# lfilipozzi/PathPlanning

Measured on AMD Instinct MI355X. Metric: hybrid_astar_plans_per_sec_1024x1024, higher is better.
Workload: dtype f64

## Files before the change

### pathplanning_amd/csrc/pp_internal.hpp

```cpp
#pragma once

#include <hip/hip_runtime.h>
#include <stdint.h>
#include <string>
#include <vector>

#include "../../include/pp_hip.h"
#include "pp_device.hpp"

namespace pph {

void set_error(const std::string& msg);
int hip_fail(hipError_t e, const char* what);

#define PP_HIP_TRY(expr)                       \
	do {                                       \
		hipError_t _e = (expr);                \
		if (_e != hipSuccess)                  \
			return pph::hip_fail(_e, #expr);   \
	} while (0)

constexpr int kMaxPrimitives = 128;
struct PrimTable {
	int n;
	double kappa[kMaxPrimitives];
	double invKappa[kMaxPrimitives];
	int8_t backward[kMaxPrimitives];
};

struct RolloutParams {
	double arcLength;
	double spatialRes, angularRes;
	ppd::Resolutions lat;
	double forwardMult, reverseMult, voronoiMult;
	float voroDiagRes;
	int headingAlias;
};

struct NonHoloDesc {
	int nx, ny, na;
	double spatialRes, angularRes, offX, offY;
	double rmin;
	float reverseCost, forwardCost, switchCost;
	double minMult;
	int negativeKRead;
};

hipError_t launch_d2_to_distance(hipStream_t s, const int32_t* d2, float* dist, int64_t n, float res);
hipError_t launch_occ_to_u8(hipStream_t s, const int32_t* occ, uint8_t* occ8, int64_t n);
hipError_t launch_check_states(hipStream_t s, const ppd::MapView& m, int64_t n, const double* poses, uint8_t* valid);
hipError_t launch_check_states_fused(hipStream_t s, const ppd::MapView& m, int64_t n, uint64_t seed, uint64_t* count);
hipError_t launch_check_arcs(hipStream_t s, const ppd::MapView& m, int64_t n, const double* from, const double* kappa, const double* length, const int32_t* dir,
	uint8_t* valid, float* last);
hipError_t launch_check_segments(hipStream_t s, const ppd::MapView& m, int64_t n, const double* from, const double* to, uint8_t* valid);
hipError_t launch_rollout(hipStream_t s, const ppd::MapView& m, const RolloutParams& rp, const PrimTable& prims, int64_t nParents, const double* parents,
	uint8_t* valid, double* pose, int32_t* key, double* cost, double* length);
hipError_t launch_rs_solve(hipStream_t s, int64_t n, const double* from, const double* to, double rmin, float rev, float fwd, float sw, int32_t* word,
	double* tuv, float* cost, double* segLength);
hipError_t launch_valid_bits(hipStream_t s, const float* dist, int64_t cells, float minSafeRadius, uint32_t* bits);
hipError_t launch_nonholo_build(hipStream_t s, const NonHoloDesc& d, double* table);
hipError_t launch_knn(hipStream_t s, int64_t nPoints, const double* pts, int64_t nQueries, const double* q, int k, int32_t* idx, double* d2);

struct WavefrontWorkspace;
int64_t wavefront_workspace_bytes(int rows, int cols);
int wavefront_resident_blocks();
hipError_t warm_up_wavefront(hipStream_t s, const ppd::MapView& m, int32_t* ctlDev);
constexpr int kSlotBits = 20;
constexpr uint32_t kSlotMask = (1u << kSlotBits) - 1u;
constexpr uint32_t kGenMask = (1u << (31 - kSlotBits)) - 1u;
struct WavefrontPublish {
	const int32_t* slotList = nullptr;
	unsigned long long* readyTail = nullptr;
	unsigned long long* ready = nullptr;
	unsigned long long readyMask = 0;
	int* goalCounter = nullptr;
	int* exitCounter = nullptr;
	unsigned long long* urgent = nullptr;
	unsigned long long* urgentHead = nullptr;
	unsigned long long urgentMask = 0;
	int* claimed = nullptr;
	const uint64_t* occBits = nullptr;
	uint32_t* tilesQueue = nullptr;
	int tilesQueueWaves = 0;
	int* tilesCtl = nullptr;
	int32_t* tilesFallback = nullptr;
	unsigned long long* tilesStats = nullptr;
	hipStream_t fallbackStream = nullptr;
	hipEvent_t fallbackEvent = nullptr;
	const int* nGoalsDev = nullptr;
	int* resetOnExit = nullptr;
	bool agentPoseLoads = false;
};
void occ_bits_dims(int rows, int cols, int& wpr, int& nWordRows);
hipError_t launch_occ_bits(hipStream_t s, const uint8_t* occ8, int rows, int cols, uint64_t* bits);
bool wavefront_tiles_supported(int rows, int cols);
int wavefront_tiles_resident_blocks(int rows, int cols);
size_t wavefront_tiles_queue_words(int rows, int cols);
hipError_t warm_up_wavefront_tiles(hipStream_t s, const ppd::MapView& m, int* ctlDev);
hipError_t launch_wavefront_tiles(hipStream_t s, const ppd::MapView& m, int nGoals, const int32_t* goalCellsDev, float* costDev, bool tiledOut, const double* goalPosesDev,
	const double* orderStartsDev, float* orderKeysDev, const WavefrontPublish& pub);
hipError_t launch_order_by_key(hipStream_t s, int n, const float* keysDev, int32_t* orderOutDev);
bool wavefront_tiles_enabled();
hipError_t launch_wavefront(hipStream_t s, const ppd::MapView& m, int nGoals, const int32_t* goalCellsDev, float* costDev, void* workspaceDev,
	int64_t workspaceBytesPerSlot, int nSlots, int32_t* errorFlagDev, unsigned long long* profDev = nullptr, bool tiledOut = false,
	const double* goalPosesDev = nullptr, bool countersZeroed = false, const double* orderStartsDev = nullptr, int32_t* orderOutDev = nullptr,
	int* doneCounterDev = nullptr, float* orderKeysDev = nullptr, const WavefrontPublish& pub = WavefrontPublish());

}

struct pp_ctx;
struct pp_map;
namespace pph {
struct GvdReference;
void gvd_reference_free(pp_map* map);
int refresh_occupancy_views(pp_map* map, hipStream_t s);
void ctx_release(pp_ctx* ctx);
void map_release(pp_map* map);
}

struct pp_ctx {
	int refs = 1;
	int device = 0;
	hipStream_t stream = nullptr;
	bool ownsStream = false;
	hipEvent_t ev0 = nullptr, ev1 = nullptr;
// ... 27 lines not shown
```

### pathplanning_amd/csrc/pp_pipeline.hpp

```cpp
#pragma once

#include <chrono>
#include <cstring>
#include <deque>
#include <unordered_map>

namespace {

__global__ void __launch_bounds__(256) k_pipe_scatter(int n, const int32_t* __restrict__ slotList, const double* __restrict__ startsIn, const double* __restrict__ goalsIn,
	const uint64_t* __restrict__ seedsIn, double* __restrict__ starts, double* __restrict__ goals, uint64_t* __restrict__ seeds, MapView m, float urgentClearance, PipeCtl* ctl,
	unsigned long long* __restrict__ urgent, unsigned long long urgentMask, int* __restrict__ claimed)
{
	const int i = (int)(blockIdx.x * blockDim.x + threadIdx.x);
	bool isUrgent = false;
	uint32_t entry = 0;
	if (i < n) {
		entry = (uint32_t)slotList[i];
		const size_t s = (size_t)(entry & pph::kSlotMask);
		for (int k = 0; k < 3; k++) {
			starts[3 * s + k] = startsIn[3 * (size_t)i + k];
			goals[3 * s + k] = goalsIn[3 * (size_t)i + k];
		}
		seeds[s] = seedsIn[i];
		if (claimed) {
// ... 574 lines not shown
		P->segmentEvents.pop_back();
	} else {
		PP_HIP_TRY(hipEventCreateWithFlags(&seg.done, hipEventDisableTiming));
	}
	struct DeadGuard {
		pp_pipeline* P;
		bool armed = true;
		~DeadGuard()
		{
			if (armed)
				P->dead = true;
		}
	} guard { P };
	P->segmentEvents.push_back(seg.done);
	int32_t* const stage = P->slotStage + P->slotListPos;
	int32_t* const listDev = P->slotLists + P->slotListPos;
	P->slotListPos += (size_t)k;
	for (int i = 0; i < k; i++) {
		const int32_t s = P->freeSlots.back();
		P->freeSlots.pop_back();
		uint32_t& gen = P->slotGen[(size_t)s];
		gen = gen >= pph::kGenMask ? 1u : gen + 1u;
		stage[i] = (int32_t)((uint32_t)s | (gen << pph::kSlotBits));
		P->slotState[(size_t)s] = 1;
		const uint64_t ticket = P->nTickets++;
		P->ticketOfSlot[(size_t)s] = ticket;
		P->slotOfTicket[ticket] = s;
		if (tickets_out)
			tickets_out[i] = ticket;
	}
	hipStream_t const w = P->wfStream[P->nextWf];
	const int wfIdx = P->nextWf;
	int32_t* const wctl = P->wfCtl[P->nextWf];
	const int fbSet = P->nextFbSet;
	P->nextFbSet = (P->nextFbSet + 1) % pp_pipeline::kFbSets;
	if (P->fbUsed[fbSet])
		PP_HIP_TRY(hipEventSynchronize(P->fbDone[fbSet]));
	int32_t* const werr = P->errFlags + P->nextWf;
	const bool tilesOn = pl->map->occBits && pph::wavefront_tiles_enabled() && pph::wavefront_tiles_supported(pl->map->desc.rows, pl->map->desc.cols);
	void* const wws = P->wfWorkspace[tilesOn ? 0 : P->nextWf];
	P->nextWf = (P->nextWf + 1) % P->nWf;
	PP_HIP_TRY(hipMemcpyAsync(listDev, stage, (size_t)k * 4, hipMemcpyHostToDevice, P->ctlStream));
	pl->args.m = pl->map->view();
	hipLaunchKernelGGL(k_pipe_scatter, dim3((k + 255) / 256), dim3(256), 0, P->ctlStream, k, listDev, starts_dev, goals_dev, seeds_dev, pl->dStarts, pl->dGoals, pl->dSeeds, pl->args.m,
		P->urgentClearance < 0.0f ? 2.0f * pl->args.m.minSafeRadius : P->urgentClearance, P->ctl, P->urgent, P->readyMask, P->claimed);
	PP_HIP_TRY(hipGetLastError());
	PP_HIP_TRY(hipEventRecord(P->evIngest, P->ctlStream));
	PP_HIP_TRY(hipStreamSynchronize(P->ctlStream));
	PP_HIP_TRY(hipStreamWaitEvent(w, P->evIngest, 0));
	pl->args.m = pl->map->view();
	pph::WavefrontPublish pub;
	pub.slotList = listDev;
	pub.readyTail = &P->ctl->readyTail;
	pub.ready = P->ready;
	pub.readyMask = P->readyMask;
	pub.goalCounter = wctl + 1;
	pub.exitCounter = wctl + 2;
	pub.claimed = P->claimed;
	pub.occBits = pl->map->occBits;
	pub.tilesCtl = P->fbCtl[fbSet];
	pub.tilesFallback = P->fbList[fbSet];
	pub.tilesQueue = P->tilesQueue[wfIdx];
	pub.tilesQueueWaves = P->tilesQueue[wfIdx] ? P->tilesQueueWaves : 0;
	pub.fallbackStream = P->fbStream;
	pub.fallbackEvent = P->fbAfterTiles[fbSet];
	if (P->urgentClearance != 0.0f) {
		pub.urgent = P->urgent;
		pub.urgentHead = &P->ctl->urgentHead;
		pub.urgentMask = P->readyMask;
	}
	const pp_pipeline::Timed tm = timed_take(P, w, 0, k);
	PP_HIP_TRY(pph::launch_wavefront(w, pl->args.m, k, nullptr, pl->costFields, wws, pl->wfBytesPerSlot, P->wfBlocks, werr, nullptr, true, pl->dGoals,
		true, nullptr, nullptr, nullptr, nullptr, pub));
	timed_done(P, w, tm);
	PP_HIP_TRY(hipEventRecord(P->fbDone[fbSet], P->fbStream));
	P->fbUsed[fbSet] = true;
	PP_HIP_TRY(hipEventRecord(seg.done, w));
	P->segmentEvents.pop_back();
	P->segments.push_back(seg);
	P->nSubmitted += (unsigned long long)k;
	*n_accepted = k;
	const int rc = pipe_launch_search(P);
	guard.armed = rc != PP_OK;
	return rc;
}

int pp_pipeline_submit(pp_pipeline* P, int32_t n_queries, const double* starts_host, const double* goals_host, const uint64_t* seeds_host, uint64_t* tickets_out, int32_t* n_accepted)
{
	if (!P || n_queries < 0 || !n_accepted || (n_queries > 0 && (!starts_host || !goals_host || !seeds_host))) {
		set_error("invalid arguments");
		return PP_ERR_INVALID;
	}
	*n_accepted = 0;
	int k = n_queries < (int)P->freeSlots.size() ? n_queries : (int)P->freeSlots.size();
	if (k == 0)
		return PP_OK;
	PP_HIP_TRY(hipSetDevice(P->pl->map->ctx->device));
	double *ds = nullptr, *dg = nullptr;
	uint64_t* dz = nullptr;
	hipError_t e = hipMalloc((void**)&ds, (size_t)k * 24);
	if (e == hipSuccess)
		e = hipMalloc((void**)&dg, (size_t)k * 24);
	if (e == hipSuccess)
		e = hipMalloc((void**)&dz, (size_t)k * 8);
	if (e == hipSuccess)
		e = hipMemcpy(ds, starts_host, (size_t)k * 24, hipMemcpyHostToDevice);
// ... 216 lines not shown
```

### pathplanning_amd/csrc/pp_wavefront_tiles.hip

```cpp
#include <cstdio>
#include "pp_internal.hpp"

#include <cstdlib>
#include <type_traits>

using namespace ppd;

namespace {

constexpr int TT = 64;
template <int TW>
struct TileShape {
	static constexpr int LS = TW + 2;
	static constexpr int LN = (TT + 2) * LS;
	static constexpr int LNP = (LN + 3) & ~3;
	typedef typename std::conditional<TW == 64, uint64_t, uint32_t>::type Mask;
};
constexpr uint32_t kInfBits = 0x7F800000u;
#ifndef PP_WF_TILES_PRIO_DEFAULT
#define PP_WF_TILES_PRIO_DEFAULT 1
#endif
#ifndef PP_WF_TILE_WIDTH_DEFAULT
#define PP_WF_TILE_WIDTH_DEFAULT 32
#endif

__device__ __forceinline__ void wave_sync()
{
	__builtin_amdgcn_fence(__ATOMIC_ACQ_REL, "wavefront");
	__builtin_amdgcn_wave_barrier();
}
__device__ __forceinline__ uint32_t from_prev_lane(uint32_t v, uint32_t first) { return (uint32_t)__builtin_amdgcn_update_dpp((int)first, (int)v, 0x138, 0xF, 0xF, false); }
__device__ __forceinline__ uint32_t from_next_lane(uint32_t v, uint32_t last) { return (uint32_t)__builtin_amdgcn_update_dpp((int)last, (int)v, 0x130, 0xF, 0xF, false); }
__device__ __forceinline__ uint64_t from_prev_lane64(uint64_t v, uint64_t first)
{
	return (uint64_t)from_prev_lane((uint32_t)v, (uint32_t)first) | ((uint64_t)from_prev_lane((uint32_t)(v >> 32), (uint32_t)(first >> 32)) << 32);
}
__device__ __forceinline__ uint64_t from_next_lane64(uint64_t v, uint64_t last)
{
	return (uint64_t)from_next_lane((uint32_t)v, (uint32_t)last) | ((uint64_t)from_next_lane((uint32_t)(v >> 32), (uint32_t)(last >> 32)) << 32);
}
__device__ __forceinline__ uint32_t mask_from_prev(uint32_t v, uint32_t first) { return from_prev_lane(v, first); }
__device__ __forceinline__ uint32_t mask_from_next(uint32_t v, uint32_t last) { return from_next_lane(v, last); }
__device__ __forceinline__ uint64_t mask_from_prev(uint64_t v, uint64_t first) { return from_prev_lane64(v, first); }
__device__ __forceinline__ uint64_t mask_from_next(uint64_t v, uint64_t last) { return from_next_lane64(v, last); }
__device__ __forceinline__ uint32_t wave_min_u32(uint32_t v)
{
	const int id = (int)0xFFFFFFFF;
	uint32_t x = v;
	x = min(x, (uint32_t)__builtin_amdgcn_update_dpp(id, (int)x, 0x111, 0xF, 0xF, false));
	x = min(x, (uint32_t)__builtin_amdgcn_update_dpp(id, (int)x, 0x112, 0xF, 0xF, false));
	x = min(x, (uint32_t)__builtin_amdgcn_update_dpp(id, (int)x, 0x114, 0xF, 0xF, false));
	x = min(x, (uint32_t)__builtin_amdgcn_update_dpp(id, (int)x, 0x118, 0xF, 0xF, false));
	x = min(x, (uint32_t)__builtin_amdgcn_update_dpp(id, (int)x, 0x142, 0xA, 0xF, false));
	x = min(x, (uint32_t)__builtin_amdgcn_update_dpp(id, (int)x, 0x143, 0xC, 0xF, false));
	return (uint32_t)__builtin_amdgcn_readlane((int)x, 63);
}
__device__ __forceinline__ float wave_min_nonneg(float v) { return __uint_as_float(wave_min_u32(__float_as_uint(v))); }

template <int TW>
__device__ __forceinline__ void tile_cell(int tiledOut, int e, int& i, int& j)
{
	if (tiledOut) {
		const int ft = e >> (2 * kFieldTileLog2), within = e & ((1 << (2 * kFieldTileLog2)) - 1);
		constexpr int perRow = TW >> kFieldTileLog2;
		i = ((ft / perRow) << kFieldTileLog2) + (within >> kFieldTileLog2);
		j = ((ft % perRow) << kFieldTileLog2) + (within & kFieldTileMask);
	} else {
		i = e / TW;
		j = e % TW;
	}
}

__global__ void __launch_bounds__(256) k_occ_bits(const uint8_t* __restrict__ occ8, int rows, int cols, int wpr, int nWordRows, uint64_t* __restrict__ bits)
{
	const int64_t w = (int64_t)blockIdx.x * 4 + (threadIdx.x >> 6);
	const int lane = threadIdx.x & 63;
	if (w >= (int64_t)nWordRows * wpr)
		return;
	const int pr = (int)(w / wpr), pw = (int)(w - (int64_t)pr * wpr);
	const int r = pr - 1, c = (pw - 1) * 64 + lane;
	bool o = true;
	if (r >= 0 && r < rows && pw >= 1 && c < cols)
		o = occ8[(int64_t)r * cols + c] != 0;
	const uint64_t b = __ballot(o);
	if (lane == 0)
		bits[w] = b;
}

struct TilesArgs {
	MapView m;
	int nGoals;
	const int32_t* goalCells;
	const double* goalPoses;
	float* costOut;
	int tiledOut;
	int* ctl;
	int32_t* fbList;
	const double* orderStarts;
	float* orderKeys;
	unsigned long long* stats;
	int forceFallbackEvery;
	int ldsPerWave;
	int prio;
	pph::WavefrontPublish pub;
};

template <int TW, bool kProf, bool kGQ>
__global__ void __launch_bounds__(512) k_wavefront_tiles(TilesArgs A)
{
	unsigned long long ph[5] = { 0, 0, 0, 0, 0 }, tl = 0;
#define TILE_STAMP(i)                                        \
	if (kProf) {                                             \
		const unsigned long long now_ = __builtin_readcyclecounter(); \
		ph[i] += now_ - tl;                                  \
		tl = now_;                                           \
	}
	typedef typename TileShape<TW>::Mask Mask;
	constexpr int LS = TileShape<TW>::LS, LNP = TileShape<TW>::LNP;
	constexpr Mask kAll = (Mask)~(Mask)0;
	extern __shared__ __attribute__((aligned(16))) uint32_t smemAll[];
	const int lane = threadIdx.x & 63;
	uint32_t* const smemRaw = smemAll + (size_t)__builtin_amdgcn_readfirstlane((int)(threadIdx.x >> 6)) * (size_t)(A.ldsPerWave >> 2);
	if (A.prio == 1)
		__builtin_amdgcn_s_setprio(1);
	else if (A.prio == 2)
		__builtin_amdgcn_s_setprio(2);
	else if (A.prio == 3)
		__builtin_amdgcn_s_setprio(3);
	const MapView& m = A.m;
	const int rows = m.rows, cols = m.cols;
	const int TR = (rows + TT - 1) / TT, TC = (cols + TW - 1) / TW, nTiles = TR * TC;
	float* const L = reinterpret_cast<float*>(smemRaw);
	const uint32_t* const Lu = smemRaw;
	uint16_t* const tqL = reinterpret_cast<uint16_t*>(L + LNP);
	const int nTileWords = (nTiles + 1) >> 1;
	uint32_t* const tqG = kGQ ? A.pub.tilesQueue + ((size_t)blockIdx.x * (blockDim.x >> 6) + (threadIdx.x >> 6)) * (size_t)nTileWords : nullptr;
	constexpr uint32_t kNotQueued = 0x7FFFu;
	auto tq_word = [&](int w) -> uint32_t {
		if (kGQ)
			return __hip_atomic_load(tqG + w, __ATOMIC_RELAXED, __HIP_MEMORY_SCOPE_AGENT);
		return reinterpret_cast<const uint32_t*>(tqL)[w];
	};
	auto tq_get = [&](int t) -> uint32_t {
		if (kGQ)
			return (uint32_t)__hip_atomic_load(reinterpret_cast<uint16_t*>(tqG) + t, __ATOMIC_RELAXED, __HIP_MEMORY_SCOPE_AGENT);
		return (uint32_t)tqL[t];
	};
	auto tq_set = [&](int t, uint32_t v) {
		if (kGQ)
			__hip_atomic_store(reinterpret_cast<uint16_t*>(tqG) + t, (uint16_t)v, __ATOMIC_RELAXED, __HIP_MEMORY_SCOPE_AGENT);
		else
			tqL[t] = (uint16_t)v;
	};
	auto tq_sync = [&]() {
		if (kGQ)
			asm volatile("s_waitcnt vmcnt(0)" ::: "memory");
		else
			wave_sync();
	};
	const float kInf = __builtin_huge_valf();
	const float kDiag = sqrtf(2.0f);
	const int64_t cells = (int64_t)rows * cols;
	const int64_t fieldElems = A.tiledOut ? (int64_t)field_tiled_elems(rows, cols) : cells;
	const uint64_t* const occW = A.pub.occBits;
	const int wpr = (cols + 63) / 64 + 2;
	auto out_index = [&](int r, int c) -> size_t { return A.tiledOut ? field_tiled_index(cols, r, c) : (size_t)r * cols + c; };

	int pendingSlot = -1;
	bool ringTurn = true;
	unsigned long long stVisits = 0, stRounds = 0, stPasses = 0, stCells = 0, stGoals = 0, stFb = 0;
	const unsigned long long t0 = A.stats ? __builtin_readcyclecounter() : 0ull;
	for (;;) {
		asm volatile("s_waitcnt vmcnt(0)" ::: "memory");
		int next = -1, st = -1;
		if (lane == 0) {
			if (pendingSlot >= 0) {
				__builtin_amdgcn_fence(__ATOMIC_RELEASE, "agent");
				asm volatile("s_waitcnt vmcnt(0)" ::: "memory");
				const unsigned long long t = __hip_atomic_fetch_add(A.pub.readyTail, 1ull, __ATOMIC_RELAXED, __HIP_MEMORY_SCOPE_AGENT);
				__hip_atomic_store(A.pub.ready + (t & A.pub.readyMask), ((t + 1ull) << 32) | (unsigned long long)(uint32_t)pendingSlot, __ATOMIC_RELAXED, __HIP_MEMORY_SCOPE_AGENT);
			}
			auto take_urgent = [&]() -> int {
				for (;;) {
					unsigned long long h = __hip_atomic_load(A.pub.urgentHead, __ATOMIC_RELAXED, __HIP_MEMORY_SCOPE_AGENT);
					const unsigned long long e = __hip_atomic_load(A.pub.urgent + (h & A.pub.urgentMask), __ATOMIC_RELAXED, __HIP_MEMORY_SCOPE_AGENT);
					if ((uint32_t)(e >> 32) != (uint32_t)(h + 1ull))
						return -1;
					if (!__hip_atomic_compare_exchange_strong(A.pub.urgentHead, &h, h + 1ull, __ATOMIC_RELAXED, __ATOMIC_RELAXED, __HIP_MEMORY_SCOPE_AGENT))
						continue;
					const int slot = (int)((uint32_t)e & pph::kSlotMask);
					int expect = (int)(((uint32_t)e >> pph::kSlotBits) << 1);
					if (__hip_atomic_compare_exchange_strong(A.pub.claimed + slot, &expect, expect | 1, __ATOMIC_RELAXED, __ATOMIC_RELAXED, __HIP_MEMORY_SCOPE_AGENT))
						return slot;
				}
			};
			if (A.pub.urgent && ringTurn)
				next = take_urgent();
			while (next < 0) {
				const int gi = atomicAdd(A.ctl, 1);
				if (gi >= A.nGoals)
					break;
				if (!A.pub.slotList) {
					next = gi;
				} else {
					const uint32_t e = (uint32_t)A.pub.slotList[gi];
					const int slot = (int)(e & pph::kSlotMask);
					int expect = (int)((e >> pph::kSlotBits) << 1);
					if (!A.pub.claimed || __hip_atomic_compare_exchange_strong(A.pub.claimed + slot, &expect, expect | 1, __ATOMIC_RELAXED, __ATOMIC_RELAXED, __HIP_MEMORY_SCOPE_AGENT))
						next = slot;
				}
			}
			ringTurn = !ringTurn;
			if (next >= 0) {
				if (A.goalPoses) {
					double px, py;
					if (A.pub.claimed) {
						px = __hip_atomic_load(A.goalPoses + 3 * (size_t)next, __ATOMIC_RELAXED, __HIP_MEMORY_SCOPE_AGENT);
						py = __hip_atomic_load(A.goalPoses + 3 * (size_t)next + 1, __ATOMIC_RELAXED, __HIP_MEMORY_SCOPE_AGENT);
					} else {
						px = A.goalPoses[3 * (size_t)next];
						py = A.goalPoses[3 * (size_t)next + 1];
					}
					int row, col;
					world_to_cell(m, px, py, row, col);
					st = inside_map(m, row, col) ? row * m.cols + col : -1;
				} else {
					st = A.goalCells[next];
				}
			}
		}
		const int g = __builtin_amdgcn_readfirstlane(next);
		const int start = __builtin_amdgcn_readfirstlane(st);
		pendingSlot = -1;
		if (g < 0)
			break;
		if (kProf)
			stGoals++;
		float* const cost = A.costOut + (int64_t)g * fieldElems;
		const int goalR = start >= 0 ? start / cols : -1, goalC = start >= 0 ? start - goalR * cols : -1;

		if (kGQ) {
			for (int w = lane; w < nTileWords; w += 64)
				__hip_atomic_store(tqG + w, kNotQueued | (kNotQueued << 16), __ATOMIC_RELAXED, __HIP_MEMORY_SCOPE_AGENT);
		} else {
			for (int t = lane; t < ((nTiles + 1) & ~1); t += 64)
				tqL[t] = (uint16_t)kNotQueued;
		}
		tq_sync();
		if (start >= 0 && lane == 0)
			tq_set((goalR / TT) * TC + goalC / TW, 0u);
		tq_sync();
		bool flagged = false;
		int visits = 0;
		const int visitBudget = 6 * nTiles + 64;

		for (;;) {
			uint32_t bestBits = kNotQueued;
			int bestT = -1;
			if (kGQ)
				asm volatile("s_waitcnt vmcnt(0)" ::: "memory");
			for (int t2 = lane; t2 < (nTiles + 1) / 2; t2 += 64) {
				const uint32_t w = tq_word(t2);
				const uint32_t lo = w & 0x7FFFu, hi = (w >> 16) & 0x7FFFu;
				if (lo < bestBits) {
					bestBits = lo;
					bestT = 2 * t2;
				}
				if (hi < bestBits) {
					bestBits = hi;
					bestT = 2 * t2 + 1;
				}
			}
			const uint32_t minBits = wave_min_u32(bestBits);
			if (minBits == kNotQueued)
				break;
			const uint64_t who = __ballot(bestBits == minBits);
			const int t = __builtin_amdgcn_readlane(bestT, (int)__builtin_ctzll(who));
			if (++visits > visitBudget) {
				flagged = true;
				break;
			}
			if (kProf)
				tl = __builtin_readcyclecounter();
			const int tr = t / TC, tc = t - tr * TC;
			const int r0 = tr * TT, c0 = tc * TW;
			auto solved = [&](int dtr, int dtc) -> bool {
				const int a = tr + dtr, b = tc + dtc;
				return a >= 0 && b >= 0 && a < TR && b < TC && (tq_get(a * TC + b) & 0x8000u);
			};
			const bool selfSolved = solved(0, 0);
			asm volatile("s_waitcnt vmcnt(0)" ::: "memory");
			auto occ_bits = [&](int prow, int cFirst) -> Mask {
				const uint64_t w = occW[(size_t)prow * wpr + (size_t)((cFirst >> 6) + 1)];
				return (Mask)(w >> (cFirst & 63));
			};
			auto occ_bit = [&](int prow, int c) -> uint32_t {
				return (uint32_t)(occW[(size_t)prow * wpr + (size_t)((c >> 6) + 1)] >> (c & 63)) & 1u;
			};
			const Mask occ = occ_bits(r0 + lane + 1, c0);
			const uint32_t occL = occ_bit(r0 + lane + 1, c0 - 1), occR = occ_bit(r0 + lane + 1, c0 + TW);
			const Mask tH = occ_bits(r0, c0), bH = occ_bits(r0 + TT + 1, c0);
			const uint32_t tHL = occ_bit(r0, c0 - 1), tHR = occ_bit(r0, c0 + TW);
			const uint32_t bHL = occ_bit(r0 + TT + 1, c0 - 1), bHR = occ_bit(r0 + TT + 1, c0 + TW);
			float hT = kInf, hB = kInf, hL = kInf, hR = kInf, hC = kInf;
			float oT = kInf, oB = kInf, oL = kInf, oR = kInf;
			{
				const int cj = c0 + lane, ri = r0 + lane;
				if (lane < TW && cj < cols) {
					if (solved(-1, 0))
						hT = cost[out_index(r0 - 1, cj)];
					if (r0 + TT < rows && solved(1, 0))
						hB = cost[out_index(r0 + TT, cj)];
				}
				if (ri < rows) {
					if (solved(0, -1))
						hL = cost[out_index(ri, c0 - 1)];
					if (c0 + TW < cols && solved(0, 1))
						hR = cost[out_index(ri, c0 + TW)];
				}
				if (lane < 4) {
					const int dr = lane < 2 ? -1 : 1, dc = (lane & 1) ? 1 : -1;
					const int rr = dr < 0 ? r0 - 1 : r0 + TT, cc = dc < 0 ? c0 - 1 : c0 + TW;
					if (rr >= 0 && rr < rows && cc >= 0 && cc < cols && solved(dr, dc))
						hC = cost[out_index(rr, cc)];
				}
				if (selfSolved) {
					if (lane < TW && cj < cols) {
						oT = cost[out_index(r0, cj)];
						if (r0 + TT - 1 < rows)
							oB = cost[out_index(r0 + TT - 1, cj)];
					}
					if (ri < rows) {
						oL = cost[out_index(ri, c0)];
						if (c0 + TW - 1 < cols)
							oR = cost[out_index(ri, c0 + TW - 1)];
					}
				}
			}
			{
				float4* const L4 = reinterpret_cast<float4*>(L);
				const float4 inf4 = make_float4(kInf, kInf, kInf, kInf);
				for (int i = lane; i < LNP / 4; i += 64)
					L4[i] = inf4;
			}
			wave_sync();
			if (lane < TW) {
				L[lane + 1] = hT;
				L[(TT + 1) * LS + lane + 1] = hB;
			}
			L[(lane + 1) * LS] = hL;
			L[(lane + 1) * LS + TW + 1] = hR;
			if (lane < 4)
				L[(lane < 2 ? 0 : (TT + 1) * LS) + ((lane & 1) ? TW + 1 : 0)] = hC;
			Mask closed = occ, cur = 0, nx1 = 0, nx2 = 0;
			const bool goalHere = goalR >= r0 && goalR < r0 + TT && goalC >= c0 && goalC < c0 + TW;
			if (goalHere && lane == goalR - r0) {
				L[(lane + 1) * LS + (goalC - c0) + 1] = 0.0f;
				closed |= (Mask)1 << (goalC - c0);
				cur = (Mask)1 << (goalC - c0);
			}
			wave_sync();
			const int hbT = hT < kInf ? (int)hT : -1, hbB = hB < kInf ? (int)hB : -1, hbL = hL < kInf ? (int)hL : -1, hbR = hR < kInf ? (int)hR : -1, hbC = hC < kInf ? (int)hC : -1;
			int kmin;
			{
				uint32_t a = 0xFFFFFFFFu;
				a = min(a, (uint32_t)hbT);
				a = min(a, (uint32_t)hbB);
				a = min(a, (uint32_t)hbL);
				a = min(a, (uint32_t)hbR);
				a = min(a, (uint32_t)hbC);
				a = wave_min_u32(a);
				kmin = goalHere ? 0 : (int)a;
			}
			if (kProf)
				stVisits++;
			TILE_STAMP(0)
			if (kmin >= 0) {
				const Mask occUp = mask_from_prev(occ, tH), occDn = mask_from_next(occ, bH);
				const Mask occWst = (Mask)(occ << 1) | (Mask)occL, occEst = (Mask)(occ >> 1) | ((Mask)occR << (TW - 1));
				const Mask bNW = occUp & occWst, bNE = occUp & occEst, bSW = occDn & occWst, bSE = occDn & occEst;
				const Mask aNW = ~bNW, aNE = ~bNE, aSW = ~bSW, aSE = ~bSE;
				int k = kmin;
				for (;;) {
					const Mask topM = (Mask)__ballot(hbT == k), botM = (Mask)__ballot(hbB == k);
					const uint32_t cm = (uint32_t)__ballot(hbC == k) & 0xFu;
					const uint32_t lr = (hbL == k ? 1u : 0u) | (hbR == k ? 2u : 0u);
					const uint32_t lrU = from_prev_lane(lr, cm & 3u), lrD = from_next_lane(lr, (cm >> 2) & 3u);
					const Mask up = mask_from_prev(cur, topM), dn = mask_from_next(cur, botM);
					const Mask mW = (Mask)(cur << 1) | (Mask)(lr & 1u), mE = (Mask)(cur >> 1) | ((Mask)(lr >> 1) << (TW - 1));
					const Mask mNW = ((Mask)(up << 1) | (Mask)(lrU & 1u)) & aNW, mNE = ((Mask)(up >> 1) | ((Mask)(lrU >> 1) << (TW - 1))) & aNE;
					const Mask mSW = ((Mask)(dn << 1) | (Mask)(lrD & 1u)) & aSW, mSE = ((Mask)(dn >> 1) | ((Mask)(lrD >> 1) << (TW - 1))) & aSE;
					Mask cand = (mW | mE | up | dn | mNW | mNE | mSW | mSE) & (Mask)~closed;
					if (kProf)
						stRounds++;
					TILE_STAMP(1)
					const float kNext2 = (float)(k + 2);
					auto settle = [&](int j, uint32_t w, uint32_t e, uint32_t n, uint32_t s, uint32_t nw, uint32_t ne, uint32_t sw, uint32_t se) -> float {
						const uint32_t minS = min(min(w, e), min(n, s));
						auto blocked = [&](Mask b) -> uint32_t {
							if constexpr (sizeof(Mask) == 4)
								return (uint32_t)__builtin_amdgcn_sbfe((int)b, (unsigned)j, 1u);
							else
								return (uint32_t)-(int32_t)((uint32_t)(b >> j) & 1u);
						};
						uint32_t minD = nw | blocked(bNW);
						minD = min(minD, ne | blocked(bNE));
						minD = min(minD, sw | blocked(bSW));
						minD = min(minD, se | blocked(bSE));
						flagged |= minS == minD;
						return minS <= minD ? __uint_as_float(minS) + 1.0f : __uint_as_float(minD) + kDiag;
					};
					while (__ballot(cand != 0)) {
						if (kProf)
							stPasses++;
						if (cand != 0) {
							const int j0 = (int)__builtin_ctzll((uint64_t)cand);
							const Mask bit0 = (Mask)1 << j0;
							cand &= (Mask)~bit0;
							const bool two = cand != 0;
							const int j1 = two ? (int)__builtin_ctzll((uint64_t)cand) : j0;
							const Mask bit1 = (Mask)1 << j1;
							cand &= (Mask)~bit1;
							const int a0 = (lane + 1) * LS + j0 + 1, a1 = (lane + 1) * LS + j1 + 1;
							const uint32_t w0 = Lu[a0 - 1], e0 = Lu[a0 + 1], n0 = Lu[a0 - LS], s0 = Lu[a0 + LS];
							const uint32_t nw0 = Lu[a0 - LS - 1], ne0 = Lu[a0 - LS + 1], sw0 = Lu[a0 + LS - 1], se0 = Lu[a0 + LS + 1];
							const uint32_t w1 = Lu[a1 - 1], e1 = Lu[a1 + 1], n1 = Lu[a1 - LS], s1 = Lu[a1 + LS];
							const uint32_t nw1 = Lu[a1 - LS - 1], ne1 = Lu[a1 - LS + 1], sw1 = Lu[a1 + LS - 1], se1 = Lu[a1 + LS + 1];
							const float v0 = settle(j0, w0, e0, n0, s0, nw0, ne0, sw0, se0);
							const float v1 = settle(j1, w1, e1, n1, s1, nw1, ne1, sw1, se1);
							L[a0] = v0;
							if (two)
								L[a1] = v1;
							closed |= bit0 | bit1;
							nx1 |= (v0 < kNext2 ? bit0 : (Mask)0) | (v1 < kNext2 ? bit1 : (Mask)0);
							nx2 |= (v0 < kNext2 ? (Mask)0 : bit0) | (v1 < kNext2 ? (Mask)0 : bit1);
							if (kProf)
								stCells += two ? 2 : 1;
						}
						wave_sync();
					}
					TILE_STAMP(2)
					cur = nx1;
					nx1 = nx2;
					nx2 = 0;
					if (__ballot(closed != kAll) == 0ull)
						break;
					if (__ballot((cur | nx1) != 0) != 0ull) {
						k++;
					} else {
						uint32_t nb = 0xFFFFFFFFu;
						nb = min(nb, hbT > k ? (uint32_t)hbT : 0xFFFFFFFFu);
						nb = min(nb, hbB > k ? (uint32_t)hbB : 0xFFFFFFFFu);
						nb = min(nb, hbL > k ? (uint32_t)hbL : 0xFFFFFFFFu);
						nb = min(nb, hbR > k ? (uint32_t)hbR : 0xFFFFFFFFu);
						nb = min(nb, hbC > k ? (uint32_t)hbC : 0xFFFFFFFFu);
						nb = wave_min_u32(nb);
						if (nb == 0xFFFFFFFFu)
							break;
						k = (int)nb;
					}
				}
			}
			wave_sync();
			{
				const int lc = lane < TW ? lane : 0;
				const float nT = lane < TW ? L[LS + lc + 1] : kInf, nB = lane < TW ? L[TT * LS + lc + 1] : kInf, nL = L[(lane + 1) * LS + 1], nR = L[(lane + 1) * LS + TW];
				auto sees = [&](float p, float q, uint32_t qOcc) -> bool { return !qOcc && (q == kInf || p < q - 0.99f); };
				const uint32_t occLU = from_prev_lane(occL, tHL), occLD = from_next_lane(occL, bHL);
				const uint32_t occRU = from_prev_lane(occR, tHR), occRD = from_next_lane(occR, bHR);
				float pN = kInf, pS = kInf, pW = kInf, pE = kInf, pNW = kInf, pNE = kInf, pSW = kInf, pSE = kInf;
				{
					const bool ch = lane < TW && __float_as_uint(nT) != __float_as_uint(oT);
					const float p = fminf(nT, oT);
					const uint32_t o0 = lc == 0 ? tHL : (uint32_t)(tH >> (lc - 1)) & 1u, o1 = (uint32_t)(tH >> lc) & 1u, o2 = lc == TW - 1 ? tHR : (uint32_t)(tH >> (lc + 1)) & 1u;
					const bool c0_ = ch && sees(p, L[lc], o0), c1_ = ch && sees(p, L[lc + 1], o1), c2_ = ch && sees(p, L[lc + 2], o2);
					if (c1_ || (lc > 0 && c0_) || (lc < TW - 1 && c2_))
						pN = p;
					if (lc == 0 && c0_)
						pNW = p;
					if (lc == TW - 1 && c2_)
						pNE = p;
				}
				{
					const bool ch = lane < TW && __float_as_uint(nB) != __float_as_uint(oB);
					const float p = fminf(nB, oB);
					const float* const Lb = L + (TT + 1) * LS;
					const uint32_t o0 = lc == 0 ? bHL : (uint32_t)(bH >> (lc - 1)) & 1u, o1 = (uint32_t)(bH >> lc) & 1u, o2 = lc == TW - 1 ? bHR : (uint32_t)(bH >> (lc + 1)) & 1u;
					const bool c0_ = ch && sees(p, Lb[lc], o0), c1_ = ch && sees(p, Lb[lc + 1], o1), c2_ = ch && sees(p, Lb[lc + 2], o2);
					if (c1_ || (lc > 0 && c0_) || (lc < TW - 1 && c2_))
						pS = p;
					if (lc == 0 && c0_)
						pSW = p;
					if (lc == TW - 1 && c2_)
						pSE = p;
				}
				{
					const bool ch = __float_as_uint(nL) != __float_as_uint(oL);
					const float p = fminf(nL, oL);
					const bool c0_ = ch && sees(p, L[lane * LS], occLU), c1_ = ch && sees(p, L[(lane + 1) * LS], occL), c2_ = ch && sees(p, L[(lane + 2) * LS], occLD);
					if (c1_ || (lane > 0 && c0_) || (lane < 63 && c2_))
						pW = p;
					if (lane == 0 && c0_)
						pNW = fminf(pNW, p);
					if (lane == 63 && c2_)
						pSW = fminf(pSW, p);
				}
				{
					const bool ch = __float_as_uint(nR) != __float_as_uint(oR);
					const float p = fminf(nR, oR);
					const bool c0_ = ch && sees(p, L[lane * LS + TW + 1], occRU), c1_ = ch && sees(p, L[(lane + 1) * LS + TW + 1], occR), c2_ = ch && sees(p, L[(lane + 2) * LS + TW + 1], occRD);
					if (c1_ || (lane > 0 && c0_) || (lane < 63 && c2_))
						pE = p;
					if (lane == 0 && c0_)
						pNE = fminf(pNE, p);
					if (lane == 63 && c2_)
						pSE = fminf(pSE, p);
				}
				const float qN = wave_min_nonneg(pN), qS = wave_min_nonneg(pS), qW = wave_min_nonneg(pW), qE = wave_min_nonneg(pE);
				const float qNW = wave_min_nonneg(pNW), qNE = wave_min_nonneg(pNE), qSW = wave_min_nonneg(pSW), qSE = wave_min_nonneg(pSE);
				if (lane < 9) {
					const int dtr = lane < 2 ? (lane == 0 ? -1 : 1) : (lane < 4 ? 0 : (lane < 6 ? -1 : (lane < 8 ? 1 : 0)));
					const int dtc = lane < 2 ? 0 : (lane < 4 ? (lane == 2 ? -1 : 1) : (lane < 8 ? ((lane & 1) ? 1 : -1) : 0));
					const float p = lane == 0 ? qN : lane == 1 ? qS : lane == 2 ? qW : lane == 3 ? qE : lane == 4 ? qNW : lane == 5 ? qNE : lane == 6 ? qSW : lane == 7 ? qSE : kInf;
					const int a = tr + dtr, b = tc + dtc;
					if (lane == 8) {
						tq_set(t, 0x8000u | kNotQueued);
					} else if (p < kInf && a >= 0 && b >= 0 && a < TR && b < TC) {
						const uint32_t bucket = p < 32766.0f ? (uint32_t)p : 32766u, old = tq_get(a * TC + b);
						if (bucket < (old & 0x7FFFu))
							tq_set(a * TC + b, (old & 0x8000u) | bucket);
					}
				}
			}
			TILE_STAMP(3)
			for (int u = 0; u < TW; u++) {
				int i, j;
				tile_cell<TW>(A.tiledOut, u * TT + lane, i, j);
				const int r = r0 + i, c = c0 + j;
				if (r < rows && c < cols)
					cost[out_index(r, c)] = L[(i + 1) * LS + j + 1];
			}
			wave_sync();
			TILE_STAMP(4)
		}
		flagged = __ballot(flagged) != 0ull;
		if (!flagged) {
			for (int t = 0; t < nTiles; t++) {
				if (tq_get(t) & 0x8000u)
					continue;
				const int tr = t / TC, tc = t - tr * TC;
				for (int u = 0; u < TW; u++) {
					int i, j;
					tile_cell<TW>(A.tiledOut, u * TT + lane, i, j);
					const int r = tr * TT + i, c = tc * TW + j;
					if (r < rows && c < cols)
						cost[out_index(r, c)] = kInf;
				}
			}
		}
		if (A.forceFallbackEvery > 0 && (g % A.forceFallbackEvery) == A.forceFallbackEvery - 1)
			flagged = true;
		if (flagged) {
			if (kProf)
				stFb++;
			if (lane == 0)
				A.fbList[atomicAdd(A.ctl + 2, 1)] = g;
			continue;
		}
		if (A.pub.ready)
			pendingSlot = g;
		if (A.orderKeys) {
			asm volatile("s_waitcnt vmcnt(0)" ::: "memory");
			if (lane == 0) {
				int row, col;
				world_to_cell(m, A.orderStarts[3 * (size_t)g], A.orderStarts[3 * (size_t)g + 1], row, col);
				float c = kInf;
				if (inside_map(m, row, col))
					c = cost[out_index(row, col)];
				__hip_atomic_store(A.orderKeys + g, c, __ATOMIC_RELAXED, __HIP_MEMORY_SCOPE_AGENT);
			}
		}
	}
	if (kProf && A.stats && lane == 0) {
		atomicAdd(A.stats + 0, stGoals);
		atomicAdd(A.stats + 1, stVisits);
		atomicAdd(A.stats + 2, stRounds);
		atomicAdd(A.stats + 3, stPasses);
		atomicAdd(A.stats + 5, stFb);
		atomicAdd(A.stats + 6, (unsigned long long)(__builtin_readcyclecounter() - t0));
		if (kProf)
			for (int i = 0; i < 5; i++)
				atomicAdd(A.stats + 8 + i, ph[i]);
	}
#undef TILE_STAMP
	if (kProf && A.stats)
		atomicAdd(A.stats + 4, stCells);
	if (lane == 0) {
		__builtin_amdgcn_fence(__ATOMIC_RELEASE, "agent");
// ... 41 lines not shown
		const char* e = getenv("PP_WF_TILE_WIDTH");
		return e && atoi(e) == 64 ? 64 : (e && atoi(e) == 32 ? 32 : PP_WF_TILE_WIDTH_DEFAULT);
	}();
	return w;
}

size_t tiles_count(int rows, int cols)
{
	const int tw = tile_width();
	return (size_t)((rows + TT - 1) / TT) * (size_t)((cols + tw - 1) / tw);
}

size_t tiles_lds_bytes(int rows, int cols, bool queueInGlobal = false)
{
	const size_t nTiles = tiles_count(rows, cols);
	return ((size_t)(tile_width() == 64 ? TileShape<64>::LNP : TileShape<32>::LNP) * 4 + (queueInGlobal ? 0 : ((nTiles + 1) & ~(size_t)1) * 2) + 15) & ~(size_t)15;
}

int waves_per_pack(size_t ldsPerWave)
{
	static const int forced = [] {
		const char* e = getenv("PP_WF_TILES_PACK");
		return e ? atoi(e) : 0;
	}();
	if (forced >= 1 && forced <= 8)
		return forced;
	int n = (int)((80 * 1024) / ldsPerWave) + 1;
	while (n > 1 && (size_t)n * ldsPerWave > 160 * 1024)
		n--;
	return n > 8 ? 8 : n;
}

void launch_tiles_kernel(hipStream_t s, int waves, TilesArgs A)
{
	const bool gq = A.pub.tilesQueue && A.pub.tilesQueueWaves > 0 && !A.stats;
	const size_t lds = tiles_lds_bytes(A.m.rows, A.m.cols, gq);
	static const bool trace = getenv("PP_WF_TILES_TRACE") != nullptr;
	if (trace && A.nGoals > 0)
		fprintf(stderr, "[tiles] launch: %d waves, tile queue in %s\n", waves, gq ? "global memory" : "LDS");
	const int pack = A.pub.ready ? waves_per_pack(lds) : 1;
	static const size_t minPackLds = [] {
		const char* e = getenv("PP_WF_TILES_PACK_KB");
		const int v = e ? atoi(e) : 82;
		return (size_t)(v < 1 ? 1 : (v > 160 ? 160 : v)) * 1024;
	}();
	const size_t packLds = pack > 1 && (size_t)pack * lds < minPackLds ? minPackLds : (size_t)pack * lds;
	A.ldsPerWave = (int)lds;
	static const int prio = [] {
		const char* e = getenv("PP_WF_TILES_PRIO");
		const int v = e ? atoi(e) : PP_WF_TILES_PRIO_DEFAULT;
		return v < 0 ? 0 : (v > 3 ? 3 : v);
	}();
	A.prio = prio;
	if (gq && waves > A.pub.tilesQueueWaves / pack * pack)
		waves = A.pub.tilesQueueWaves / pack * pack;
	const int grid = (waves + pack - 1) / pack;
	static const bool attr = [] {
		(void)hipFuncSetAttribute(reinterpret_cast<const void*>(k_wavefront_tiles<64, false, false>), hipFuncAttributeMaxDynamicSharedMemorySize, 160 * 1024);
		(void)hipFuncSetAttribute(reinterpret_cast<const void*>(k_wavefront_tiles<32, false, false>), hipFuncAttributeMaxDynamicSharedMemorySize, 160 * 1024);
		(void)hipFuncSetAttribute(reinterpret_cast<const void*>(k_wavefront_tiles<64, true, false>), hipFuncAttributeMaxDynamicSharedMemorySize, 160 * 1024);
		(void)hipFuncSetAttribute(reinterpret_cast<const void*>(k_wavefront_tiles<32, true, false>), hipFuncAttributeMaxDynamicSharedMemorySize, 160 * 1024);
		(void)hipFuncSetAttribute(reinterpret_cast<const void*>(k_wavefront_tiles<64, false, true>), hipFuncAttributeMaxDynamicSharedMemorySize, 160 * 1024);
		(void)hipFuncSetAttribute(reinterpret_cast<const void*>(k_wavefront_tiles<32, false, true>), hipFuncAttributeMaxDynamicSharedMemorySize, 160 * 1024);
		return true;
	}();
	(void)attr;
	if (tile_width() == 64) {
		if (A.stats)
			hipLaunchKernelGGL((k_wavefront_tiles<64, true, false>), dim3(grid), dim3(64 * pack), packLds, s, A);
		else if (gq)
			hipLaunchKernelGGL((k_wavefront_tiles<64, false, true>), dim3(grid), dim3(64 * pack), packLds, s, A);
		else
			hipLaunchKernelGGL((k_wavefront_tiles<64, false, false>), dim3(grid), dim3(64 * pack), packLds, s, A);
	} else {
		if (A.stats)
			hipLaunchKernelGGL((k_wavefront_tiles<32, true, false>), dim3(grid), dim3(64 * pack), packLds, s, A);
		else if (gq)
			hipLaunchKernelGGL((k_wavefront_tiles<32, false, true>), dim3(grid), dim3(64 * pack), packLds, s, A);
		else
			hipLaunchKernelGGL((k_wavefront_tiles<32, false, false>), dim3(grid), dim3(64 * pack), packLds, s, A);
	}
}

}

namespace pph {

void occ_bits_dims(int rows, int cols, int& wpr, int& nWordRows)
{
	wpr = (cols + TT - 1) / TT + 2;
	nWordRows = (rows + TT - 1) / TT * TT + 2;
}

hipError_t launch_occ_bits(hipStream_t s, const uint8_t* occ8, int rows, int cols, uint64_t* bits)
{
	int wpr, nWordRows;
	occ_bits_dims(rows, cols, wpr, nWordRows);
	const int64_t words = (int64_t)wpr * nWordRows;
	hipLaunchKernelGGL(k_occ_bits, dim3((unsigned)((words + 3) / 4)), dim3(256), 0, s, occ8, rows, cols, wpr, nWordRows, bits);
	return hipGetLastError();
}

bool wavefront_tiles_supported(int rows, int cols)
{
	return tiles_lds_bytes(rows, cols) <= 64 * 1024;
}
// ... 80 lines not shown
```

Baseline: 36550.

## Add fast unblocked settle path and ready-queue priority backoff to tiled wavefront

The tile settle loop now builds candidate masks with a cheap dilation when no diagonal-blocked cells are involved, and only takes the full per-direction corner-cutting path when one is. Tie detection is moved into an accumulator checked once per goal, and closed/next-bucket bookkeeping is done once per round rather than per pass. Separately, a wave lowers its scheduling priority to zero when the ready queue's backlog (tail minus head) exceeds a threshold, so consumer kernels can drain it. This trades extra branching and an atomic read per goal for fewer ALU operations per settle and better overlap with downstream stages.

```diff
diff --git a/pathplanning_amd/csrc/pp_internal.hpp b/pathplanning_amd/csrc/pp_internal.hpp
--- a/pathplanning_amd/csrc/pp_internal.hpp
+++ b/pathplanning_amd/csrc/pp_internal.hpp
@@ -71,6 +71,7 @@
 struct WavefrontPublish {
 	const int32_t* slotList = nullptr;
 	unsigned long long* readyTail = nullptr;
+	const unsigned long long* readyHead = nullptr;
 	unsigned long long* ready = nullptr;
 	unsigned long long readyMask = 0;
 	int* goalCounter = nullptr;
diff --git a/pathplanning_amd/csrc/pp_pipeline.hpp b/pathplanning_amd/csrc/pp_pipeline.hpp
--- a/pathplanning_amd/csrc/pp_pipeline.hpp
+++ b/pathplanning_amd/csrc/pp_pipeline.hpp
@@ -650,6 +650,7 @@
 	pph::WavefrontPublish pub;
 	pub.slotList = listDev;
 	pub.readyTail = &P->ctl->readyTail;
+	pub.readyHead = &P->ctl->readyHead;
 	pub.ready = P->ready;
 	pub.readyMask = P->readyMask;
 	pub.goalCounter = wctl + 1;
diff --git a/pathplanning_amd/csrc/pp_wavefront_tiles.hip b/pathplanning_amd/csrc/pp_wavefront_tiles.hip
--- a/pathplanning_amd/csrc/pp_wavefront_tiles.hip
+++ b/pathplanning_amd/csrc/pp_wavefront_tiles.hip
@@ -19,6 +19,9 @@
 constexpr uint32_t kInfBits = 0x7F800000u;
 #ifndef PP_WF_TILES_PRIO_DEFAULT
 #define PP_WF_TILES_PRIO_DEFAULT 1
+#endif
+#ifndef PP_WF_TILES_BACKOFF_DEFAULT
+#define PP_WF_TILES_BACKOFF_DEFAULT 4096
 #endif
 #ifndef PP_WF_TILE_WIDTH_DEFAULT
 #define PP_WF_TILE_WIDTH_DEFAULT 32
@@ -102,6 +105,7 @@
 	int forceFallbackEvery;
 	int ldsPerWave;
 	int prio;
+	int backoff;
 	pph::WavefrontPublish pub;
 };
 
@@ -121,12 +125,16 @@
 	extern __shared__ __attribute__((aligned(16))) uint32_t smemAll[];
 	const int lane = threadIdx.x & 63;
 	uint32_t* const smemRaw = smemAll + (size_t)__builtin_amdgcn_readfirstlane((int)(threadIdx.x >> 6)) * (size_t)(A.ldsPerWave >> 2);
-	if (A.prio == 1)
-		__builtin_amdgcn_s_setprio(1);
-	else if (A.prio == 2)
-		__builtin_amdgcn_s_setprio(2);
-	else if (A.prio == 3)
-		__builtin_amdgcn_s_setprio(3);
+	auto set_prio = [&]() {
+		if (A.prio == 1)
+			__builtin_amdgcn_s_setprio(1);
+		else if (A.prio == 2)
+			__builtin_amdgcn_s_setprio(2);
+		else if (A.prio == 3)
+			__builtin_amdgcn_s_setprio(3);
+	};
+	set_prio();
+	bool backedOff = false;
 	const MapView& m = A.m;
 	const int rows = m.rows, cols = m.cols;
 	const int TR = (rows + TT - 1) / TT, TC = (cols + TW - 1) / TW, nTiles = TR * TC;
@@ -172,7 +180,7 @@
 	const unsigned long long t0 = A.stats ? __builtin_readcyclecounter() : 0ull;
 	for (;;) {
 		asm volatile("s_waitcnt vmcnt(0)" ::: "memory");
-		int next = -1, st = -1;
+		int next = -1, st = -1, lowPrio = 0;
 		if (lane == 0) {
 			if (pendingSlot >= 0) {
 				__builtin_amdgcn_fence(__ATOMIC_RELEASE, "agent");
@@ -196,6 +204,7 @@
 			};
 			if (A.pub.urgent && ringTurn)
 				next = take_urgent();
+			const bool urgentGoal = next >= 0;
 			while (next < 0) {
 				const int gi = atomicAdd(A.ctl, 1);
 				if (gi >= A.nGoals)
@@ -211,6 +220,11 @@
 				}
 			}
 			ringTurn = !ringTurn;
+			if (next >= 0 && A.backoff > 0 && !urgentGoal) {
+				const unsigned long long tail = __hip_atomic_load(A.pub.readyTail, __ATOMIC_RELAXED, __HIP_MEMORY_SCOPE_AGENT);
+				const unsigned long long head = __hip_atomic_load(A.pub.readyHead, __ATOMIC_RELAXED, __HIP_MEMORY_SCOPE_AGENT);
+				lowPrio = tail > head + (unsigned long long)A.backoff;
+			}
 			if (next >= 0) {
 				if (A.goalPoses) {
 					double px, py;
@@ -234,6 +248,13 @@
 		pendingSlot = -1;
 		if (g < 0)
 			break;
+		if (A.backoff > 0 && (__builtin_amdgcn_readfirstlane(lowPrio) != 0) != backedOff) {
+			backedOff = !backedOff;
+			if (backedOff)
+				__builtin_amdgcn_s_setprio(0);
+			else
+				set_prio();
+		}
 		if (kProf)
 			stGoals++;
 		float* const cost = A.costOut + (int64_t)g * fieldElems;
@@ -251,6 +272,7 @@
 			tq_set((goalR / TT) * TC + goalC / TW, 0u);
 		tq_sync();
 		bool flagged = false;
+		uint32_t tieAcc = ~0u;
 		int visits = 0;
 		const int visitBudget = 6 * nTiles + 64;
 
@@ -352,7 +374,7 @@
 			L[(lane + 1) * LS + TW + 1] = hR;
 			if (lane < 4)
 				L[(lane < 2 ? 0 : (TT + 1) * LS) + ((lane & 1) ? TW + 1 : 0)] = hC;
-			Mask closed = occ, cur = 0, nx1 = 0, nx2 = 0;
+			Mask closed = occ, cur = 0, nx1 = 0;
 			const bool goalHere = goalR >= r0 && goalR < r0 + TT && goalC >= c0 && goalC < c0 + TW;
 			if (goalHere && lane == goalR - r0) {
 				L[(lane + 1) * LS + (goalC - c0) + 1] = 0.0f;
@@ -379,70 +401,85 @@
 				const Mask occUp = mask_from_prev(occ, tH), occDn = mask_from_next(occ, bH);
 				const Mask occWst = (Mask)(occ << 1) | (Mask)occL, occEst = (Mask)(occ >> 1) | ((Mask)occR << (TW - 1));
 				const Mask bNW = occUp & occWst, bNE = occUp & occEst, bSW = occDn & occWst, bSE = occDn & occEst;
-				const Mask aNW = ~bNW, aNE = ~bNE, aSW = ~bSW, aSE = ~bSE;
+				const Mask bAny = bNW | bNE | bSW | bSE;
 				int k = kmin;
 				for (;;) {
 					const Mask topM = (Mask)__ballot(hbT == k), botM = (Mask)__ballot(hbB == k);
 					const uint32_t cm = (uint32_t)__ballot(hbC == k) & 0xFu;
-					const uint32_t lr = (hbL == k ? 1u : 0u) | (hbR == k ? 2u : 0u);
-					const uint32_t lrU = from_prev_lane(lr, cm & 3u), lrD = from_next_lane(lr, (cm >> 2) & 3u);
-					const Mask up = mask_from_prev(cur, topM), dn = mask_from_next(cur, botM);
-					const Mask mW = (Mask)(cur << 1) | (Mask)(lr & 1u), mE = (Mask)(cur >> 1) | ((Mask)(lr >> 1) << (TW - 1));
-					const Mask mNW = ((Mask)(up << 1) | (Mask)(lrU & 1u)) & aNW, mNE = ((Mask)(up >> 1) | ((Mask)(lrU >> 1) << (TW - 1))) & aNE;
-					const Mask mSW = ((Mask)(dn << 1) | (Mask)(lrD & 1u)) & aSW, mSE = ((Mask)(dn >> 1) | ((Mask)(lrD >> 1) << (TW - 1))) & aSE;
-					Mask cand = (mW | mE | up | dn | mNW | mNE | mSW | mSE) & (Mask)~closed;
+					const bool inL = hbL == k, inR = hbR == k;
+					const Mask rowD = (Mask)(cur | (Mask)(cur << 1) | (Mask)(cur >> 1)) | (inL ? (Mask)1 : (Mask)0) | (inR ? (Mask)1 << (TW - 1) : (Mask)0);
+					const Mask topD = (Mask)(topM | (Mask)(topM << 1) | (Mask)(topM >> 1)) | (Mask)(cm & 1u) | ((Mask)((cm >> 1) & 1u) << (TW - 1));
+					const Mask botD = (Mask)(botM | (Mask)(botM << 1) | (Mask)(botM >> 1)) | (Mask)((cm >> 2) & 1u) | ((Mask)((cm >> 3) & 1u) << (TW - 1));
+					Mask cand = (rowD | mask_from_prev(rowD, topD) | mask_from_next(rowD, botD)) & (Mask)~closed;
+					const bool slow = __ballot((cand & bAny) != 0) != 0ull;
+					if (slow) {
+						const uint32_t lr = (inL ? 1u : 0u) | (inR ? 2u : 0u);
+						const uint32_t lrU = from_prev_lane(lr, cm & 3u), lrD = from_next_lane(lr, (cm >> 2) & 3u);
+						const Mask up = mask_from_prev(cur, topM), dn = mask_from_next(cur, botM);
+						const Mask mW = (Mask)(cur << 1) | (Mask)(lr & 1u), mE = (Mask)(cur >> 1) | ((Mask)(lr >> 1) << (TW - 1));
+						const Mask mNW = ((Mask)(up << 1) | (Mask)(lrU & 1u)) & (Mask)~bNW, mNE = ((Mask)(up >> 1) | ((Mask)(lrU >> 1) << (TW - 1))) & (Mask)~bNE;
+						const Mask mSW = ((Mask)(dn << 1) | (Mask)(lrD & 1u)) & (Mask)~bSW, mSE = ((Mask)(dn >> 1) | ((Mask)(lrD >> 1) << (TW - 1))) & (Mask)~bSE;
+						cand = (mW | mE | up | dn | mNW | mNE | mSW | mSE) & (Mask)~closed;
+					}
+					const Mask settled = cand;
 					if (kProf)
 						stRounds++;
 					TILE_STAMP(1)
 					const float kNext2 = (float)(k + 2);
-					auto settle = [&](int j, uint32_t w, uint32_t e, uint32_t n, uint32_t s, uint32_t nw, uint32_t ne, uint32_t sw, uint32_t se) -> float {
-						const uint32_t minS = min(min(w, e), min(n, s));
-						auto blocked = [&](Mask b) -> uint32_t {
-							if constexpr (sizeof(Mask) == 4)
-								return (uint32_t)__builtin_amdgcn_sbfe((int)b, (unsigned)j, 1u);
-							else
-								return (uint32_t)-(int32_t)((uint32_t)(b >> j) & 1u);
+					Mask lo = 0;
+					auto passes = [&](auto withBlocked) {
+						auto settle = [&](int j, uint32_t w, uint32_t e, uint32_t n, uint32_t s, uint32_t nw, uint32_t ne, uint32_t sw, uint32_t se) -> float {
+							const uint32_t minS = min(min(w, e), min(n, s));
+							uint32_t minD;
+							if constexpr (decltype(withBlocked)::value) {
+								auto blocked = [&](Mask b) -> uint32_t {
+									if constexpr (sizeof(Mask) == 4)
+										return (uint32_t)__builtin_amdgcn_sbfe((int)b, (unsigned)j, 1u);
+									else
+										return (uint32_t)-(int32_t)((uint32_t)(b >> j) & 1u);
+								};
+								minD = nw | blocked(bNW);
+								minD = min(minD, ne | blocked(bNE));
+								minD = min(minD, sw | blocked(bSW));
+								minD = min(minD, se | blocked(bSE));
+							} else {
+								minD = min(min(nw, ne), min(sw, se));
+							}
+							tieAcc = min(tieAcc, minS ^ minD);
+							return minS <= minD ? __uint_as_float(minS) + 1.0f : __uint_as_float(minD) + kDiag;
 						};
-						uint32_t minD = nw | blocked(bNW);
-						minD = min(minD, ne | blocked(bNE));
-						minD = min(minD, sw | blocked(bSW));
-						minD = min(minD, se | blocked(bSE));
-						flagged |= minS == minD;
-						return minS <= minD ? __uint_as_float(minS) + 1.0f : __uint_as_float(minD) + kDiag;
+						while (__ballot(cand != 0)) {
+							if (kProf)
+								stPasses++;
+							if (cand != 0) {
+								const int j0 = (int)__builtin_ctzll((uint64_t)cand);
+								const int j1 = (int)(sizeof(Mask) * 8 - 1) - (sizeof(Mask) == 4 ? (int)__builtin_clz((uint32_t)cand) : (int)__builtin_clzll((uint64_t)cand));
+								const Mask bit0 = (Mask)1 << j0, bit1 = (Mask)1 << j1;
+								cand &= (Mask)~(bit0 | bit1);
+								const int a0 = (lane + 1) * LS + j0 + 1, a1 = (lane + 1) * LS + j1 + 1;
+								const uint32_t w0 = Lu[a0 - 1], e0 = Lu[a0 + 1], n0 = Lu[a0 - LS], s0 = Lu[a0 + LS];
+								const uint32_t nw0 = Lu[a0 - LS - 1], ne0 = Lu[a0 - LS + 1], sw0 = Lu[a0 + LS - 1], se0 = Lu[a0 + LS + 1];
+								const uint32_t w1 = Lu[a1 - 1], e1 = Lu[a1 + 1], n1 = Lu[a1 - LS], s1 = Lu[a1 + LS];
+								const uint32_t nw1 = Lu[a1 - LS - 1], ne1 = Lu[a1 - LS + 1], sw1 = Lu[a1 + LS - 1], se1 = Lu[a1 + LS + 1];
+								const float v0 = settle(j0, w0, e0, n0, s0, nw0, ne0, sw0, se0);
+								const float v1 = settle(j1, w1, e1, n1, s1, nw1, ne1, sw1, se1);
+								L[a0] = v0;
+								L[a1] = v1;
+								lo |= (v0 < kNext2 ? bit0 : (Mask)0) | (v1 < kNext2 ? bit1 : (Mask)0);
+								if (kProf)
+									stCells += j1 != j0 ? 2 : 1;
+							}
+							wave_sync();
+						}
 					};
-					while (__ballot(cand != 0)) {
-						if (kProf)
-							stPasses++;
-						if (cand != 0) {
-							const int j0 = (int)__builtin_ctzll((uint64_t)cand);
-							const Mask bit0 = (Mask)1 << j0;
-							cand &= (Mask)~bit0;
-							const bool two = cand != 0;
-							const int j1 = two ? (int)__builtin_ctzll((uint64_t)cand) : j0;
-							const Mask bit1 = (Mask)1 << j1;
-							cand &= (Mask)~bit1;
-							const int a0 = (lane + 1) * LS + j0 + 1, a1 = (lane + 1) * LS + j1 + 1;
-							const uint32_t w0 = Lu[a0 - 1], e0 = Lu[a0 + 1], n0 = Lu[a0 - LS], s0 = Lu[a0 + LS];
-							const uint32_t nw0 = Lu[a0 - LS - 1], ne0 = Lu[a0 - LS + 1], sw0 = Lu[a0 + LS - 1], se0 = Lu[a0 + LS + 1];
-							const uint32_t w1 = Lu[a1 - 1], e1 = Lu[a1 + 1], n1 = Lu[a1 - LS], s1 = Lu[a1 + LS];
-							const uint32_t nw1 = Lu[a1 - LS - 1], ne1 = Lu[a1 - LS + 1], sw1 = Lu[a1 + LS - 1], se1 = Lu[a1 + LS + 1];
-							const float v0 = settle(j0, w0, e0, n0, s0, nw0, ne0, sw0, se0);
-							const float v1 = settle(j1, w1, e1, n1, s1, nw1, ne1, sw1, se1);
-							L[a0] = v0;
-							if (two)
-								L[a1] = v1;
-							closed |= bit0 | bit1;
-							nx1 |= (v0 < kNext2 ? bit0 : (Mask)0) | (v1 < kNext2 ? bit1 : (Mask)0);
-							nx2 |= (v0 < kNext2 ? (Mask)0 : bit0) | (v1 < kNext2 ? (Mask)0 : bit1);
-							if (kProf)
-								stCells += two ? 2 : 1;
-						}
-						wave_sync();
-					}
+					if (slow)
+						passes(std::true_type());
+					else
+						passes(std::false_type());
 					TILE_STAMP(2)
-					cur = nx1;
-					nx1 = nx2;
-					nx2 = 0;
+					closed |= settled;
+					cur = nx1 | lo;
+					nx1 = settled & (Mask)~lo;
 					if (__ballot(closed != kAll) == 0ull)
 						break;
 					if (__ballot((cur | nx1) != 0) != 0ull) {
@@ -543,7 +580,7 @@
 			wave_sync();
 			TILE_STAMP(4)
 		}
-		flagged = __ballot(flagged) != 0ull;
+		flagged = __ballot(flagged || tieAcc == 0u) != 0ull;
 		if (!flagged) {
 			for (int t = 0; t < nTiles; t++) {
 				if (tq_get(t) & 0x8000u)
@@ -691,6 +728,12 @@
 		return v < 0 ? 0 : (v > 3 ? 3 : v);
 	}();
 	A.prio = prio;
+	static const int backoff = [] {
+		const char* e = getenv("PP_WF_TILES_BACKOFF");
+		const int v = e ? atoi(e) : PP_WF_TILES_BACKOFF_DEFAULT;
+		return v < 0 ? 0 : v;
+	}();
+	A.backoff = A.pub.readyTail && A.pub.readyHead && prio > 0 ? backoff : 0;
 	if (gq && waves > A.pub.tilesQueueWaves / pack * pack)
 		waves = A.pub.tilesQueueWaves / pack * pack;
 	const int grid = (waves + pack - 1) / pack;
```

Measured after the change: 35890, median of 2. -1.8%, worse.
